# AIM-Harvard/pyradiomics

Measured on NVIDIA H100. Metric: voxels/s full-texture voxel-based, higher is better.
Workload: dtype f64

## Files before the change

### pyradiomics_b200/csrc/glcm_kernels.cuh

```cuda
#pragma once
#include "glcm_fast.cuh"
#include "voxel_tiles.cuh"

#ifndef RB_DYN_SHARED
#define RB_DYN_SHARED(type, name) extern __shared__ type name[]
#endif

namespace rb {

struct GlcmTask {
  long long vi;
  uint8_t slot;
  uint8_t n_ok;
  uint8_t count;
  uint8_t cls;
  float unused;
};

constexpr int GF_LZ_SMEM_BYTES = LZ_NARR * 18 * 128 * (int)sizeof(double);
constexpr int glcm_phaseA_smem_bytes(int nt) { return 27 * nt * (int)(sizeof(uint32_t) + sizeof(uint8_t)); }
template <int KIND> struct SolveKind;
template <> struct SolveKind<0> { static constexpr int lo = 0, hi = 6, minb = 4; };
template <> struct SolveKind<1> { static constexpr int lo = 7, hi = GF_DENSE_MAX_CLS, minb = 2; };
template <> struct SolveKind<2> { static constexpr int lo = GF_DENSE_MAX_CLS + 1, hi = GF_NCLS - 1, minb = 2; };

__device__ __forceinline__ void glcm_task_window(const uint8_t* __restrict__ lev, const VoxParams& P, long long vi, bool live,
                                                 uint8_t* w) {
  const int z = (int)(vi / P.sz), rem = (int)(vi % P.sz), y = rem / (int)P.sy, x = rem % (int)P.sy;
  load_window27(lev, P, z, y, x, vi, live, w, 1);
}

template <int N>
__device__ __forceinline__ void solve_group(const uint8_t* __restrict__ lev, const VoxParams& P, const GlcmSolveTables& T,
                                            const GlcmTask* __restrict__ queue, double* __restrict__ res,
                                            const uint16_t* order, unsigned base, int begin, int end) {
  for (int b0 = begin; b0 < end; b0 += 128) {
    const int i = b0 + (int)threadIdx.x;
    const bool live = i < end;
    const unsigned k = base + order[live ? i : begin];
    const GlcmTask e = queue[k];
    uint8_t w[27];
    glcm_task_window(lev, P, e.vi, live, w);
    uint32_t W7[7];
    glcm_pack_window(w, 1, W7);
    bool ok;
    const double r = glcm_small_solve<N, true>(w, 1, W7, T, e.slot, &ok, live);
    if (live) res[k] = ok ? r : NAN;
  }
}

template <int N>
__device__ __forceinline__ void lanczos_group(const uint8_t* __restrict__ lev, const VoxParams& P, const GlcmSolveTables& T,
                                              const GlcmTask* __restrict__ queue, double* __restrict__ res,
                                              const uint16_t* order, unsigned base, int begin, int end, double* scratch) {
  for (int b0 = begin; b0 < end; b0 += 128) {
    const int i = b0 + (int)threadIdx.x;
    if (b0 + (int)(threadIdx.x & ~31u) >= end) break;
    const bool live = i < end;
    const unsigned k = base + order[live ? i : begin];
    const GlcmTask e = queue[k];
    uint8_t w[27];
    glcm_task_window(lev, P, e.vi, live, w);
    int n = 0;
    double r = e.slot <= 2 ? glcm_lanczos_task<N>(w, 1, T, e.slot, scratch + threadIdx.x, 128, &n, live) : 1.0;
    if (N == 18 && n == 19) r = 1.0;
    if (live) res[k] = r;
  }
}

template <int KIND>
__global__ void __launch_bounds__(128, SolveKind<KIND>::minb)
glcm_fast_solve_kernel(const uint8_t* __restrict__ lev, const __grid_constant__ VoxParams P,
                       const GlcmFastTables* __restrict__ Tg, const GlcmTask* __restrict__ queue,
                       const unsigned* __restrict__ qcount, double* __restrict__ res, int only) {
  __shared__ GlcmSolveTables T;
  if (threadIdx.x == 0) glcm_solve_tables_from(*Tg, T);
  __syncthreads();
  const unsigned n = *qcount;
  constexpr int TILE = 4096;
  constexpr int LO = SolveKind<KIND>::lo, KC = SolveKind<KIND>::hi - SolveKind<KIND>::lo + 1;
  __shared__ uint16_t order[TILE];
  __shared__ int bucket[GF_NCLS];
  __shared__ uint16_t cnt[KC][128];
  const unsigned long long per_wave = (unsigned long long)gridDim.x * TILE;
  const unsigned ntiles = KIND == 2 ? gridDim.x * (unsigned)((n + per_wave - 1) / per_wave) : (n + TILE - 1) / TILE;
  for (unsigned tile = blockIdx.x; tile < ntiles; tile += gridDim.x) {
    const unsigned base = KIND == 2 ? (unsigned)((unsigned long long)n * tile / ntiles) : tile * TILE;
    const unsigned tend = KIND == 2 ? (unsigned)((unsigned long long)n * (tile + 1) / ntiles)
                                    : (n - base < (unsigned)TILE ? n : base + TILE);
#pragma unroll
    for (int c = 0; c < KC; c++) cnt[c][threadIdx.x] = 0;
    if (threadIdx.x < GF_NCLS) bucket[threadIdx.x] = 0;
    uint8_t mycls[TILE / 128];
#pragma unroll
    for (int j = 0; j < TILE / 128; j++) {
      const unsigned k = base + j * 128 + threadIdx.x;
      mycls[j] = k < tend ? queue[k].cls : GF_NCLS;
      const int c = (int)mycls[j] - LO;
      if (c >= 0 && c < KC) cnt[c][threadIdx.x]++;
    }
    __syncthreads();
    if ((int)threadIdx.x < KC) {
      int run = 0;
      for (int t = 0; t < 128; t++) { const int v = cnt[threadIdx.x][t]; cnt[threadIdx.x][t] = (uint16_t)run; run += v; }
      bucket[LO + threadIdx.x] = run;
    }
    __syncthreads();
    int cstart[KC];
    {
      int run = 0;
#pragma unroll
      for (int c = 0; c < KC; c++) { cstart[c] = run; run += bucket[LO + c]; }
    }
    __syncthreads();
    if ((int)threadIdx.x < KC) bucket[LO + threadIdx.x] += cstart[threadIdx.x];
#pragma unroll
    for (int j = 0; j < TILE / 128; j++) {
      const int c = (int)mycls[j] - LO;
      if (c >= 0 && c < KC) {
        int cs = 0;
#pragma unroll
        for (int q = 0; q < KC; q++) if (q == c) cs = cstart[q];
        order[cs + cnt[c][threadIdx.x]++] = (uint16_t)(j * 128 + threadIdx.x);
      }
    }
    __syncthreads();
    if (KIND == 2) {
      RB_DYN_SHARED(double, lz_scratch);
      const int e14 = bucket[12], e16 = bucket[14], e18 = bucket[15];
      if (!only || only == 18) lanczos_group<18>(lev, P, T, queue, res, order, base, e16, e18, lz_scratch);
      if (!only || only == 16) lanczos_group<16>(lev, P, T, queue, res, order, base, e14, e16, lz_scratch);
      if (!only || only == 14) lanczos_group<14>(lev, P, T, queue, res, order, base, 0, e14, lz_scratch);
    } else {
      if (KIND == 0) {
        if (!only || only == 4) solve_group<4>(lev, P, T, queue, res, order, base, 0, bucket[2]);
        if (!only || only == 6) solve_group<6>(lev, P, T, queue, res, order, base, bucket[2], bucket[4]);
        if (!only || only == 8) solve_group<8>(lev, P, T, queue, res, order, base, bucket[4], bucket[6]);
      } else {
        if (!only || only == 10) solve_group<10>(lev, P, T, queue, res, order, base, 0, bucket[8]);
        if (!only || only == 12) solve_group<12>(lev, P, T, queue, res, order, base, bucket[8], bucket[GF_DENSE_MAX_CLS]);
      }
    }
    __syncthreads();
  }
}

template <bool FULL, int NT, typename OutT>
__device__ __forceinline__ void glcm_phaseA_voxel(const uint8_t* w, uint32_t* eq, const GlcmFastTables& T, const VoxParams& P,
                                                  const ChunkVoxel& v, bool store, OutT* __restrict__ out, long long fstride,
                                                  GlcmTask* __restrict__ queue, unsigned* __restrict__ qcount,
                                                  double* __restrict__ mcc_part, long long t) {
  double f[GLCM_NF];
  int n_ok = 0;
  unsigned long long tcls = 0;
  const uint32_t tasks = glcm_fast_voxel_phaseA<FULL>(w, NT, eq, NT, T, P, f, &n_ok, &tcls);
  if (!store) return;
#pragma unroll
  for (int k = 0; k < GLCM_NF; k++) store_map(out + k * fstride + v.oi, f[k]);
  if constexpr (!std::is_same<OutT, double>::value) {
    if (tasks) mcc_part[t] = f[G_MCC];
  }
  if (tasks) {
    const int k = __popc(tasks);
    unsigned q = atomicAdd(qcount, (unsigned)k);
    bool first = true;
    for (uint32_t m = tasks; m; m &= m - 1, q++) {
      GlcmTask e;
      e.vi = v.vi; e.slot = (uint8_t)(__ffs((int)m) - 1); e.n_ok = (uint8_t)n_ok; e.count = first ? (uint8_t)k : 0;
      e.cls = (uint8_t)(tcls >> (GF_CLS_BITS * e.slot) & (GF_NCLS - 1)); e.unused = 0.f;
      queue[q] = e;
      first = false;
    }
  }
}

template <int MINB, int NT, typename OutT>
__global__ void __launch_bounds__(NT, MINB)
glcm_fast_kernel(const uint8_t* __restrict__ lev, const uint8_t* __restrict__ centers,
                 const __grid_constant__ VoxParams P, const GlcmFastTables* __restrict__ Tg,
                 OutT* __restrict__ out, long long fstride, int z0, int z1, int out_z0,
                 GlcmTask* __restrict__ queue, unsigned* __restrict__ qcount, double* __restrict__ mcc_part = nullptr) {
  __shared__ GlcmFastTables T;
  __shared__ unsigned defer[2 * NT];
  __shared__ unsigned ndefer;
  RB_DYN_SHARED(uint32_t, eqbuf);
  uint8_t* const wbuf = reinterpret_cast<uint8_t*>(eqbuf + 27 * NT);
  copy_tables_to_shared<NT>(T, Tg);
  if (threadIdx.x == 0) ndefer = 0;
  __syncthreads();
  uint8_t* const w = &wbuf[threadIdx.x];
  uint32_t* const eq = &eqbuf[threadIdx.x];
  full_window_tiles<NT>((long long)(z1 - z0) * P.Y * P.X, defer, ndefer,
    [&](long long t, bool live, auto defer_it) {
      const long long plane = (long long)P.Y * P.X;
      const ChunkVoxel v = chunk_voxel(P, plane, z0, out_z0, t, live);
      const bool center = live && chunk_center(lev, centers, plane, v);
      if (load_window27(lev, P, v.z, v.y, v.x, v.vi, center, w, NT)) {
        glcm_phaseA_voxel<true, NT>(w, eq, T, P, v, true, out, fstride, queue, qcount, mcc_part, t);
      } else if (center) {
        defer_it();
      } else if (live) {
#pragma unroll
        for (int k = 0; k < GLCM_NF; k++) store_map(out + k * fstride + v.oi, P.init_value);
      }
    },
    [&](auto entry, bool live) {
      const long long plane = (long long)P.Y * P.X;
      const long long t = live ? entry() : 0;
      const ChunkVoxel v = chunk_voxel(P, plane, z0, out_z0, t, live);
      load_window27(lev, P, v.z, v.y, v.x, v.vi, live && chunk_center(lev, centers, plane, v), w, NT);
      glcm_phaseA_voxel<false, NT>(w, eq, T, P, v, live, out, fstride, queue, qcount, mcc_part, t);
    });
}


template <typename OutT>
__global__ void __launch_bounds__(256)
glcm_fast_finish_kernel(const __grid_constant__ VoxParams P, const GlcmTask* __restrict__ queue,
                        const unsigned* __restrict__ qcount, const double* __restrict__ res,
                        OutT* __restrict__ mcc_map , int out_z0,
                        const double* __restrict__ mcc_part = nullptr, int za = 0) {
  const unsigned n = *qcount;
  const long long plane = (long long)P.Y * P.X;
  for (unsigned k = blockIdx.x * blockDim.x + threadIdx.x; k < n; k += gridDim.x * blockDim.x) {
    const GlcmTask e = queue[k];
    if (!e.count) continue;
    double add = 0;
    for (int j = 0; j < e.count; j++) add += res[k + j];
    const long long oi = e.vi - (long long)out_z0 * plane;
    if constexpr (std::is_same<OutT, double>::value) mcc_map[oi] += add / e.n_ok;
    else {
      const double mcc = mcc_part[e.vi - (long long)za * plane] + add / e.n_ok;
      store_map(mcc_map + oi, mcc);
    }
  }
}

}
```

### pyradiomics_b200/csrc/voxel_fast.cu

```cuda
#include <map>
#include <mutex>
#include <vector>

#include "common.cuh"
#define RB_GLCM_BLOCK_SYNC 1
#include "glcm_fast.cuh"
#include "glcm_kernels.cuh"
#include "glrlm_fast.cuh"
#include "small_fast.cuh"
#include "host_common.hpp"

namespace rb {

struct GlcmQueue {
  GlcmTask* q = nullptr; double* res = nullptr; unsigned* count = nullptr; size_t cap = 0;
  double* mcc = nullptr; size_t mcc_cap = 0;
  std::mutex mu;
};
static std::mutex g_queue_mu;
static std::map<std::pair<int, cudaStream_t>, GlcmQueue> g_queue_cache;
int glcm_release_queues() {
  int dev = 0;
  if (cudaGetDevice(&dev) != cudaSuccess) return RB_ERR_CUDA;
  std::vector<std::unique_lock<std::mutex>> held;
  std::vector<GlcmQueue*> mine;
  {
    std::lock_guard<std::mutex> lk(g_queue_mu);
    for (auto& kv : g_queue_cache)
      if (kv.first.first == dev) mine.push_back(&kv.second);
  }
  for (GlcmQueue* Q : mine) held.emplace_back(Q->mu);
  cudaDeviceSynchronize();
  for (GlcmQueue* Q : mine) {
    cudaFree(Q->q); cudaFree(Q->res); cudaFree(Q->count); cudaFree(Q->mcc);
    Q->q = nullptr; Q->res = nullptr; Q->count = nullptr; Q->mcc = nullptr; Q->cap = Q->mcc_cap = 0;
  }
  return RB_OK;
}
static GlcmQueue* glcm_queue(cudaStream_t st, size_t need, size_t mcc_need, std::unique_lock<std::mutex>& lk) {
  int dev = 0;
  if (cudaGetDevice(&dev) != cudaSuccess) return nullptr;
  GlcmQueue* entry;
  {
    std::lock_guard<std::mutex> mlk(g_queue_mu);
    entry = &g_queue_cache[{dev, st}];
  }
  lk = std::unique_lock<std::mutex>(entry->mu);
  GlcmQueue& Q = *entry;
  if (!Q.count && cudaMalloc(&Q.count, sizeof(unsigned)) != cudaSuccess) return nullptr;
  if (Q.cap < need) {
    if (Q.q) { cudaStreamSynchronize(st); cudaFree(Q.q); cudaFree(Q.res); Q.q = nullptr; Q.res = nullptr; Q.cap = 0; }
    if (cudaMalloc(&Q.q, need * sizeof(GlcmTask)) != cudaSuccess) return nullptr;
    if (cudaMalloc(&Q.res, need * sizeof(double)) != cudaSuccess) { cudaFree(Q.q); Q.q = nullptr; return nullptr; }
    Q.cap = need;
  }
  if (Q.mcc_cap < mcc_need) {
    if (Q.mcc) { cudaStreamSynchronize(st); cudaFree(Q.mcc); Q.mcc = nullptr; Q.mcc_cap = 0; }
    if (cudaMalloc(&Q.mcc, mcc_need * sizeof(double)) != cudaSuccess) return nullptr;
    Q.mcc_cap = mcc_need;
  }
  return &Q;
}

template <typename OutT>
static int glcm_fast_run(const uint8_t* l8, const uint8_t* centers, const VoxParams& P, OutT* out, long long fstride,
                         int z0, int z1, int out_z0, cudaStream_t st) {
  const GlcmFastTables* T = device_table<GlcmFastTables>([&](GlcmFastTables& h) { glcm_fast_build_tables(h, P.Ng); }, P.Ng);
  if (!T) return fail(RB_ERR_CUDA, "could not build the GLCM table block on the device");
  const long long plane = (long long)P.Y * P.X;
  if ((long long)(z1 - z0) * plane <= 0) return RB_OK;
  if (P.sy != P.X || P.sz != plane) return fail(RB_ERR_ARG, "GLCM fast path expects a contiguous level volume");
  const int sms = sm_count();
  const long long max_entries = 48ll << 20;
  int zchunk = (int)(max_entries / (plane * GF_NA));
  if (zchunk < 1) zchunk = 1;
  if (zchunk > z1 - z0) zchunk = z1 - z0;
  const int nchunks = (z1 - z0 + zchunk - 1) / zchunk;
  zchunk = (z1 - z0 + nchunks - 1) / nchunks;
  constexpr bool f64 = std::is_same<OutT, double>::value;
  std::unique_lock<std::mutex> qlk;
  GlcmQueue* Q = glcm_queue(st, (size_t)zchunk * plane * GF_NA, f64 ? 0 : (size_t)zchunk * plane, qlk);
  if (!Q) return fail(RB_ERR_NOMEM, "could not allocate the GLCM eigen-task queue");
  constexpr int NT = 512;
  const int smem = glcm_phaseA_smem_bytes(NT);
  RB_CUDA(set_max_dynamic_smem(glcm_fast_kernel<1, NT, OutT>, smem));
  RB_CUDA(set_max_dynamic_smem(glcm_fast_solve_kernel<2>, GF_LZ_SMEM_BYTES));
  for (int za = z0; za < z1; za += zchunk) {
    const int zb = za + zchunk < z1 ? za + zchunk : z1;
    RB_CUDA(cudaMemsetAsync(Q->count, 0, sizeof(unsigned), st));
    int grid = 0;
    RB_CUDA(resident_grid(glcm_fast_kernel<1, NT, OutT>, NT, smem, (long long)(zb - za) * plane, grid));
    glcm_fast_kernel<1, NT, OutT><<<grid, NT, smem, st>>>(l8, centers, P, T, out, fstride, za, zb, out_z0, Q->q, Q->count,
                                                         Q->mcc);
    RB_LAUNCH_CHECK();
    glcm_fast_solve_kernel<0><<<sms * 8, 128, 0, st>>>(l8, P, T, Q->q, Q->count, Q->res, 0);
    for (int g = 10; g <= 12; g += 2) glcm_fast_solve_kernel<1><<<sms * 8, 128, 0, st>>>(l8, P, T, Q->q, Q->count, Q->res, g);
    for (int g = 18; g >= 14; g -= 2)
      glcm_fast_solve_kernel<2><<<sms * 2, 128, GF_LZ_SMEM_BYTES, st>>>(l8, P, T, Q->q, Q->count, Q->res, g);
    RB_LAUNCH_CHECK();
    glcm_fast_finish_kernel<OutT><<<sms * 8, 256, 0, st>>>(P, Q->q, Q->count, Q->res, out + (long long)G_MCC * fstride,
                                                           out_z0, Q->mcc, za);
    RB_LAUNCH_CHECK();
  }
  return RB_OK;
}

template <typename OutT>
__global__ void __launch_bounds__(128)
glrlm_fast_kernel(const uint8_t* __restrict__ lev, const uint8_t* __restrict__ centers,
                  const __grid_constant__ VoxParams P, const GlrlmFastTables* __restrict__ Tg,
                  OutT* __restrict__ out, long long fstride, int z0, int z1, int out_z0) {
  __shared__ GlrlmFastTables T;
  copy_tables_to_shared(T, Tg);
  __syncthreads();
  const long long plane = (long long)P.Y * P.X;
  const long long total = (long long)(z1 - z0) * plane;
  for (long long t = (long long)blockIdx.x * blockDim.x + threadIdx.x; t < total; t += (long long)gridDim.x * blockDim.x) {
    const ChunkVoxel v = chunk_voxel(P, plane, z0, out_z0, t);
    if (!chunk_center(lev, centers, plane, v)) {
#pragma unroll
      for (int k = 0; k < GLRLM_NF; k++) store_map(out + k * fstride + v.oi, P.init_value);
      continue;
    }
    int wl[27];
    load_window27(lev, P, v.z, v.y, v.x, v.vi, true, wl, 1);
    double f[GLRLM_NF];
    glrlm_fast_voxel(wl, T, f);
#pragma unroll
    for (int k = 0; k < GLRLM_NF; k++) store_map(out + k * fstride + v.oi, f[k]);
  }
}

template <typename OutT>
static int glrlm_fast_run(const uint8_t* l8, const uint8_t* centers, const VoxParams& P, OutT* out, long long fstride,
                          int z0, int z1, int out_z0, cudaStream_t st) {
  const GlrlmFastTables* T = device_table<GlrlmFastTables>(glrlm_fast_build_tables);
  if (!T) return fail(RB_ERR_CUDA, "could not build the GLRLM table block on the device");
  const long long total = (long long)(z1 - z0) * P.Y * P.X;
  if (total <= 0) return RB_OK;
  glrlm_fast_kernel<<<grid_for(total, 128, 32), 128, 0, st>>>(l8, centers, P, T, out, fstride, z0, z1, out_z0);
  RB_LAUNCH_CHECK();
  return RB_OK;
}

template <int CLS> struct TileClass;
template <> struct TileClass<C_GLSZM> {
  static constexpr int NF = GLSZM_NF, NT = 128, MINB = 4;
  struct Scratch { unsigned long long mg[13 * NT]; };
  template <bool FULL>
  static __device__ __forceinline__ void body(const int* wl, const SmallFastTables& T, int, Scratch& s, int tid, double* f) {
    glszm_fast_body<FULL>(wl, T, f, s.mg + tid, NT);
  }
};
template <> struct TileClass<C_GLDM> {
  static constexpr int NF = GLDM_NF, NT = 256, MINB = 2;
  struct Scratch {};
  template <bool FULL>
  static __device__ __forceinline__ void body(const int* wl, const SmallFastTables& T, int alpha, Scratch&, int, double* f) {
    gldm_fast_body<FULL>(wl, alpha, T, f);
  }
};
template <> struct TileClass<C_NGTDM> {
  static constexpr int NF = NGTDM_NF, NT = 128, MINB = 4;
  struct Scratch { double ns[27 * NT]; int pk[27 * NT]; };
  template <bool FULL>
  static __device__ __forceinline__ void body(const int* wl, const SmallFastTables& T, int, Scratch& s, int tid, double* f) {
    ngtdm_fast_body<FULL>(wl, T, f, s.pk + tid, s.ns + tid, NT);
  }
};

template <int CLS, int NT, int MINB, typename OutT>
__global__ void __launch_bounds__(NT, MINB)
tiles_fast_kernel(const uint8_t* __restrict__ lev, const uint8_t* __restrict__ centers, const __grid_constant__ VoxParams P,
                  const SmallFastTables* __restrict__ Tg, OutT* __restrict__ out, long long fstride,
                  int z0, int z1, int out_z0) {
  using K = TileClass<CLS>;
  static_assert(NT == K::NT && MINB == K::MINB, "the scratch is laid out for the class's block size");
  __shared__ SmallFastTables T;
  __shared__ typename K::Scratch scr;
  __shared__ long long defer[2 * NT];
  __shared__ unsigned ndefer;
  copy_tables_to_shared<NT>(T, Tg);
  const int tid = threadIdx.x;
  if (tid == 0) ndefer = 0;
  __syncthreads();
  const long long plane = (long long)P.Y * P.X;
  full_window_tiles<NT>((long long)(z1 - z0) * plane, defer, ndefer,
    [&](long long t, bool live, auto defer_it) {
      if (!live) return;
      const ChunkVoxel v = chunk_voxel(P, plane, z0, out_z0, t);
      const bool is_center = chunk_center(lev, centers, plane, v);
      int wl[27];
      const bool full = load_window27(lev, P, v.z, v.y, v.x, v.vi, is_center, wl, 1);
      if (full) {
        double f[K::NF];
        K::template body<true>(wl, T, P.alpha, scr, tid, f);
#pragma unroll
        for (int k = 0; k < K::NF; k++) store_map(out + k * fstride + v.oi, f[k]);
      } else if (is_center) {
        defer_it();
      } else {
#pragma unroll
        for (int k = 0; k < K::NF; k++) store_map(out + k * fstride + v.oi, P.init_value);
      }
    },
    [&](auto entry, bool live) {
      if (!live) return;
      const ChunkVoxel v = chunk_voxel(P, plane, z0, out_z0, entry());
      int wl[27];
      load_window27(lev, P, v.z, v.y, v.x, v.vi, true, wl, 1);
      double f[K::NF];
      K::template body<false>(wl, T, P.alpha, scr, tid, f);
#pragma unroll
      for (int k = 0; k < K::NF; k++) store_map(out + k * fstride + v.oi, f[k]);
    });
}

template <int CLS, typename OutT>
static int tiles_fast_run(const uint8_t* l8, const uint8_t* centers, const VoxParams& P, OutT* out, long long fstride,
                          int z0, int z1, int out_z0, cudaStream_t st) {
  using K = TileClass<CLS>;
  const SmallFastTables* T = device_table<SmallFastTables>(small_fast_build_tables);
  if (!T) return fail(RB_ERR_CUDA, "could not build the table block on the device");
  const long long total = (long long)(z1 - z0) * P.Y * P.X;
  if (total <= 0) return RB_OK;
  int grid = 0;
  RB_CUDA(resident_grid(tiles_fast_kernel<CLS, K::NT, K::MINB, OutT>, K::NT, 0, total, grid));
  tiles_fast_kernel<CLS, K::NT, K::MINB, OutT><<<grid, K::NT, 0, st>>>(l8, centers, P, T, out, fstride, z0, z1, out_z0);
  RB_LAUNCH_CHECK();
  return RB_OK;
}

template <typename OutT>
static int fast_run(int cls, const uint8_t* l8, const uint8_t* centers, const VoxParams& P, OutT* out, long long fstride,
                    int z0, int z1, int out_z0, cudaStream_t st) {
  switch (cls) {
    case C_GLCM: return glcm_fast_run(l8, centers, P, out, fstride, z0, z1, out_z0, st);
    case C_GLRLM: return glrlm_fast_run(l8, centers, P, out, fstride, z0, z1, out_z0, st);
    case C_GLSZM: return tiles_fast_run<C_GLSZM>(l8, centers, P, out, fstride, z0, z1, out_z0, st);
    case C_GLDM: return tiles_fast_run<C_GLDM>(l8, centers, P, out, fstride, z0, z1, out_z0, st);
    default: return tiles_fast_run<C_NGTDM>(l8, centers, P, out, fstride, z0, z1, out_z0, st);
  }
}

int voxel_fast_launch(int cls, const void* lev, const uint8_t* centers, const VoxParams& P, void* out, bool out_f32,
                      long long fstride, int z0, int z1, int out_z0, cudaStream_t st) {
  const uint8_t* l8 = (const uint8_t*)lev;
  if (out_f32) return fast_run(cls, l8, centers, P, (float*)out, fstride, z0, z1, out_z0, st);
  return fast_run(cls, l8, centers, P, (double*)out, fstride, z0, z1, out_z0, st);
}

}
```

Measured before the change: 295.4 million.

## Replace tiled bucket sort in GLCM solve kernels with per-block ring-buffer stream compaction

```diff
diff --git a/pyradiomics_b200/csrc/glcm_kernels.cuh b/pyradiomics_b200/csrc/glcm_kernels.cuh
--- a/pyradiomics_b200/csrc/glcm_kernels.cuh
+++ b/pyradiomics_b200/csrc/glcm_kernels.cuh
@@ -20,9 +20,9 @@
 constexpr int GF_LZ_SMEM_BYTES = LZ_NARR * 18 * 128 * (int)sizeof(double);
 constexpr int glcm_phaseA_smem_bytes(int nt) { return 27 * nt * (int)(sizeof(uint32_t) + sizeof(uint8_t)); }
 template <int KIND> struct SolveKind;
-template <> struct SolveKind<0> { static constexpr int lo = 0, hi = 6, minb = 4; };
-template <> struct SolveKind<1> { static constexpr int lo = 7, hi = GF_DENSE_MAX_CLS, minb = 2; };
-template <> struct SolveKind<2> { static constexpr int lo = GF_DENSE_MAX_CLS + 1, hi = GF_NCLS - 1, minb = 2; };
+template <> struct SolveKind<0> { static constexpr int minb = 4, N[3] = {4, 6, 8}, clo[4] = {0, 3, 5, 7}; };
+template <> struct SolveKind<1> { static constexpr int minb = 2, N[2] = {10, 12}, clo[3] = {7, 9, GF_DENSE_MAX_CLS + 1}; };
+template <> struct SolveKind<2> { static constexpr int minb = 2, N[3] = {14, 16, 18}, clo[4] = {11, 13, 15, GF_NCLS}; };
 
 __device__ __forceinline__ void glcm_task_window(const uint8_t* __restrict__ lev, const VoxParams& P, long long vi, bool live,
                                                  uint8_t* w) {
@@ -30,41 +30,87 @@
   load_window27(lev, P, z, y, x, vi, live, w, 1);
 }
 
+__device__ __forceinline__ unsigned block_uniform_ballot(bool p) {
+#ifdef RB_EMULATE_BLOCK
+  __shared__ bool vote[128];
+  vote[threadIdx.x] = p;
+  __syncthreads();
+  unsigned m = 0;
+  for (unsigned l = 0; l < 32; l++) m |= (unsigned)vote[(threadIdx.x & ~31u) + l] << l;
+  __syncthreads();
+  return m;
+#else
+  return __ballot_sync(0xffffffffu, p);
+#endif
+}
+
+constexpr int GF_SOLVE_SPAN = 16;
+constexpr int GF_RING = GF_SOLVE_SPAN * 128 + 128;
 template <int N>
-__device__ __forceinline__ void solve_group(const uint8_t* __restrict__ lev, const VoxParams& P, const GlcmSolveTables& T,
+__device__ __forceinline__ void solve_round(const uint8_t* __restrict__ lev, const VoxParams& P, const GlcmSolveTables& T,
                                             const GlcmTask* __restrict__ queue, double* __restrict__ res,
-                                            const uint16_t* order, unsigned base, int begin, int end) {
-  for (int b0 = begin; b0 < end; b0 += 128) {
-    const int i = b0 + (int)threadIdx.x;
-    const bool live = i < end;
-    const unsigned k = base + order[live ? i : begin];
-    const GlcmTask e = queue[k];
-    uint8_t w[27];
-    glcm_task_window(lev, P, e.vi, live, w);
+                                            const unsigned* ring, unsigned head, unsigned cnt, double* scratch) {
+  const bool live = threadIdx.x < cnt;
+  if (N > 12 && (threadIdx.x & ~31u) >= cnt) return;
+  const unsigned k = ring[(head + (live ? threadIdx.x : 0u)) % GF_RING];
+  const GlcmTask e = queue[k];
+  uint8_t w[27];
+  glcm_task_window(lev, P, e.vi, live, w);
+  if constexpr (N <= 12) {
     uint32_t W7[7];
     glcm_pack_window(w, 1, W7);
     bool ok;
     const double r = glcm_small_solve<N, true>(w, 1, W7, T, e.slot, &ok, live);
     if (live) res[k] = ok ? r : NAN;
-  }
-}
-
-template <int N>
-__device__ __forceinline__ void lanczos_group(const uint8_t* __restrict__ lev, const VoxParams& P, const GlcmSolveTables& T,
-                                              const GlcmTask* __restrict__ queue, double* __restrict__ res,
-                                              const uint16_t* order, unsigned base, int begin, int end, double* scratch) {
-  for (int b0 = begin; b0 < end; b0 += 128) {
-    const int i = b0 + (int)threadIdx.x;
-    if (b0 + (int)(threadIdx.x & ~31u) >= end) break;
-    const bool live = i < end;
-    const unsigned k = base + order[live ? i : begin];
-    const GlcmTask e = queue[k];
-    uint8_t w[27];
-    glcm_task_window(lev, P, e.vi, live, w);
+  } else {
     int n = 0;
     double r = e.slot <= 2 ? glcm_lanczos_task<N>(w, 1, T, e.slot, scratch + threadIdx.x, 128, &n, live) : 1.0;
     if (N == 18 && n == 19) r = 1.0;
     if (live) res[k] = r;
+  }
+}
+
+template <int KIND, int G>
+__device__ __forceinline__ void solve_stream(const uint8_t* __restrict__ lev, const VoxParams& P, const GlcmSolveTables& T,
+                                             const GlcmTask* __restrict__ queue, double* __restrict__ res,
+                                             unsigned beg, unsigned end, unsigned* ring, unsigned (*wcnt)[4],
+                                             double* scratch) {
+  constexpr int lo = SolveKind<KIND>::clo[G], hi = SolveKind<KIND>::clo[G + 1];
+  const unsigned lane = threadIdx.x & 31u, warp = threadIdx.x >> 5;
+  unsigned head = 0, fill = 0;
+  for (unsigned s0 = beg;; s0 += GF_SOLVE_SPAN * 128) {
+    const bool last = s0 >= end;
+    if (!last) {
+      bool mine[GF_SOLVE_SPAN];
+#pragma unroll
+      for (int j = 0; j < GF_SOLVE_SPAN; j++) {
+        const unsigned k = s0 + j * 128 + threadIdx.x;
+        const int c = k < end ? (int)queue[k].cls : -1;
+        mine[j] = c >= lo && c < hi;
+      }
+      unsigned vote[GF_SOLVE_SPAN];
+#pragma unroll
+      for (int j = 0; j < GF_SOLVE_SPAN; j++) {
+        vote[j] = block_uniform_ballot(mine[j]);
+        if (lane == 0) wcnt[j][warp] = __popc(vote[j]);
+      }
+      __syncthreads();
+#pragma unroll
+      for (int j = 0; j < GF_SOLVE_SPAN; j++) {
+        unsigned before = 0, total = 0;
+#pragma unroll
+        for (unsigned q = 0; q < 4; q++) { const unsigned v = wcnt[j][q]; total += v; before += q < warp ? v : 0; }
+        if (mine[j]) ring[(head + fill + before + __popc(vote[j] & ((1u << lane) - 1))) % GF_RING] = s0 + j * 128 + threadIdx.x;
+        fill += total;
+      }
+    }
+    __syncthreads();
+    while (fill >= 128 || (last && fill)) {
+      const unsigned cnt = fill < 128 ? fill : 128;
+      solve_round<SolveKind<KIND>::N[G]>(lev, P, T, queue, res, ring, head, cnt, scratch);
+      head += cnt; fill -= cnt;
+    }
+    if (last) break;
   }
 }
 
@@ -74,74 +120,25 @@
                        const GlcmFastTables* __restrict__ Tg, const GlcmTask* __restrict__ queue,
                        const unsigned* __restrict__ qcount, double* __restrict__ res, int only) {
   __shared__ GlcmSolveTables T;
+  __shared__ unsigned ring[GF_RING];
+  __shared__ unsigned wcnt[GF_SOLVE_SPAN][4];
   if (threadIdx.x == 0) glcm_solve_tables_from(*Tg, T);
-  __syncthreads();
   const unsigned n = *qcount;
-  constexpr int TILE = 4096;
-  constexpr int LO = SolveKind<KIND>::lo, KC = SolveKind<KIND>::hi - SolveKind<KIND>::lo + 1;
-  __shared__ uint16_t order[TILE];
-  __shared__ int bucket[GF_NCLS];
-  __shared__ uint16_t cnt[KC][128];
-  const unsigned long long per_wave = (unsigned long long)gridDim.x * TILE;
-  const unsigned ntiles = KIND == 2 ? gridDim.x * (unsigned)((n + per_wave - 1) / per_wave) : (n + TILE - 1) / TILE;
-  for (unsigned tile = blockIdx.x; tile < ntiles; tile += gridDim.x) {
-    const unsigned base = KIND == 2 ? (unsigned)((unsigned long long)n * tile / ntiles) : tile * TILE;
-    const unsigned tend = KIND == 2 ? (unsigned)((unsigned long long)n * (tile + 1) / ntiles)
-                                    : (n - base < (unsigned)TILE ? n : base + TILE);
-#pragma unroll
-    for (int c = 0; c < KC; c++) cnt[c][threadIdx.x] = 0;
-    if (threadIdx.x < GF_NCLS) bucket[threadIdx.x] = 0;
-    uint8_t mycls[TILE / 128];
-#pragma unroll
-    for (int j = 0; j < TILE / 128; j++) {
-      const unsigned k = base + j * 128 + threadIdx.x;
-      mycls[j] = k < tend ? queue[k].cls : GF_NCLS;
-      const int c = (int)mycls[j] - LO;
-      if (c >= 0 && c < KC) cnt[c][threadIdx.x]++;
-    }
-    __syncthreads();
-    if ((int)threadIdx.x < KC) {
-      int run = 0;
-      for (int t = 0; t < 128; t++) { const int v = cnt[threadIdx.x][t]; cnt[threadIdx.x][t] = (uint16_t)run; run += v; }
-      bucket[LO + threadIdx.x] = run;
-    }
-    __syncthreads();
-    int cstart[KC];
-    {
-      int run = 0;
-#pragma unroll
-      for (int c = 0; c < KC; c++) { cstart[c] = run; run += bucket[LO + c]; }
-    }
-    __syncthreads();
-    if ((int)threadIdx.x < KC) bucket[LO + threadIdx.x] += cstart[threadIdx.x];
-#pragma unroll
-    for (int j = 0; j < TILE / 128; j++) {
-      const int c = (int)mycls[j] - LO;
-      if (c >= 0 && c < KC) {
-        int cs = 0;
-#pragma unroll
-        for (int q = 0; q < KC; q++) if (q == c) cs = cstart[q];
-        order[cs + cnt[c][threadIdx.x]++] = (uint16_t)(j * 128 + threadIdx.x);
-      }
-    }
-    __syncthreads();
-    if (KIND == 2) {
-      RB_DYN_SHARED(double, lz_scratch);
-      const int e14 = bucket[12], e16 = bucket[14], e18 = bucket[15];
-      if (!only || only == 18) lanczos_group<18>(lev, P, T, queue, res, order, base, e16, e18, lz_scratch);
-      if (!only || only == 16) lanczos_group<16>(lev, P, T, queue, res, order, base, e14, e16, lz_scratch);
-      if (!only || only == 14) lanczos_group<14>(lev, P, T, queue, res, order, base, 0, e14, lz_scratch);
-    } else {
-      if (KIND == 0) {
-        if (!only || only == 4) solve_group<4>(lev, P, T, queue, res, order, base, 0, bucket[2]);
-        if (!only || only == 6) solve_group<6>(lev, P, T, queue, res, order, base, bucket[2], bucket[4]);
-        if (!only || only == 8) solve_group<8>(lev, P, T, queue, res, order, base, bucket[4], bucket[6]);
-      } else {
-        if (!only || only == 10) solve_group<10>(lev, P, T, queue, res, order, base, 0, bucket[8]);
-        if (!only || only == 12) solve_group<12>(lev, P, T, queue, res, order, base, bucket[8], bucket[GF_DENSE_MAX_CLS]);
-      }
-    }
-    __syncthreads();
+  const unsigned beg = (unsigned)((unsigned long long)n * blockIdx.x / gridDim.x);
+  const unsigned end = (unsigned)((unsigned long long)n * (blockIdx.x + 1) / gridDim.x);
+  __syncthreads();
+  if constexpr (KIND == 0) {
+    if (!only || only == 4) solve_stream<0, 0>(lev, P, T, queue, res, beg, end, ring, wcnt, nullptr);
+    if (!only || only == 6) solve_stream<0, 1>(lev, P, T, queue, res, beg, end, ring, wcnt, nullptr);
+    if (!only || only == 8) solve_stream<0, 2>(lev, P, T, queue, res, beg, end, ring, wcnt, nullptr);
+  } else if constexpr (KIND == 1) {
+    if (!only || only == 10) solve_stream<1, 0>(lev, P, T, queue, res, beg, end, ring, wcnt, nullptr);
+    if (!only || only == 12) solve_stream<1, 1>(lev, P, T, queue, res, beg, end, ring, wcnt, nullptr);
+  } else {
+    RB_DYN_SHARED(double, lz_scratch);
+    if (!only || only == 18) solve_stream<2, 2>(lev, P, T, queue, res, beg, end, ring, wcnt, lz_scratch);
+    if (!only || only == 16) solve_stream<2, 1>(lev, P, T, queue, res, beg, end, ring, wcnt, lz_scratch);
+    if (!only || only == 14) solve_stream<2, 0>(lev, P, T, queue, res, beg, end, ring, wcnt, lz_scratch);
   }
 }
 
diff --git a/pyradiomics_b200/csrc/voxel_fast.cu b/pyradiomics_b200/csrc/voxel_fast.cu
--- a/pyradiomics_b200/csrc/voxel_fast.cu
+++ b/pyradiomics_b200/csrc/voxel_fast.cu
@@ -85,6 +85,11 @@
   const int smem = glcm_phaseA_smem_bytes(NT);
   RB_CUDA(set_max_dynamic_smem(glcm_fast_kernel<1, NT, OutT>, smem));
   RB_CUDA(set_max_dynamic_smem(glcm_fast_solve_kernel<2>, GF_LZ_SMEM_BYTES));
+  const long long qmax = (long long)zchunk * plane * GF_NA;
+  int sgrid[3] = {0, 0, 0};
+  RB_CUDA(resident_grid(glcm_fast_solve_kernel<0>, 128, 0, qmax, sgrid[0]));
+  RB_CUDA(resident_grid(glcm_fast_solve_kernel<1>, 128, 0, qmax, sgrid[1]));
+  RB_CUDA(resident_grid(glcm_fast_solve_kernel<2>, 128, GF_LZ_SMEM_BYTES, qmax, sgrid[2]));
   for (int za = z0; za < z1; za += zchunk) {
     const int zb = za + zchunk < z1 ? za + zchunk : z1;
     RB_CUDA(cudaMemsetAsync(Q->count, 0, sizeof(unsigned), st));
@@ -93,10 +98,10 @@
     glcm_fast_kernel<1, NT, OutT><<<grid, NT, smem, st>>>(l8, centers, P, T, out, fstride, za, zb, out_z0, Q->q, Q->count,
                                                          Q->mcc);
     RB_LAUNCH_CHECK();
-    glcm_fast_solve_kernel<0><<<sms * 8, 128, 0, st>>>(l8, P, T, Q->q, Q->count, Q->res, 0);
-    for (int g = 10; g <= 12; g += 2) glcm_fast_solve_kernel<1><<<sms * 8, 128, 0, st>>>(l8, P, T, Q->q, Q->count, Q->res, g);
+    glcm_fast_solve_kernel<0><<<sgrid[0], 128, 0, st>>>(l8, P, T, Q->q, Q->count, Q->res, 0);
+    for (int g = 10; g <= 12; g += 2) glcm_fast_solve_kernel<1><<<sgrid[1], 128, 0, st>>>(l8, P, T, Q->q, Q->count, Q->res, g);
     for (int g = 18; g >= 14; g -= 2)
-      glcm_fast_solve_kernel<2><<<sms * 2, 128, GF_LZ_SMEM_BYTES, st>>>(l8, P, T, Q->q, Q->count, Q->res, g);
+      glcm_fast_solve_kernel<2><<<sgrid[2], 128, GF_LZ_SMEM_BYTES, st>>>(l8, P, T, Q->q, Q->count, Q->res, g);
     RB_LAUNCH_CHECK();
     glcm_fast_finish_kernel<OutT><<<sms * 8, 256, 0, st>>>(P, Q->q, Q->count, Q->res, out + (long long)G_MCC * fstride,
                                                            out_z0, Q->mcc, za);
```

Result: no change. 297.6 million (median of 6 runs) (+0.7%).
